# GoatWu/AdaLog

Measured on AMD Instinct MI355X. Metric: calib_images_per_sec, higher is better.
Workload: dtype bf16

## Files before the change

### adalog_amd/csrc/gemm_k_avw.inc

```
struct AvwCand { float s, inv, lo, hi; };
__device__ __forceinline__ uint4 avw_gen8(const v4u& xa, const v4u& xb, const AvwCand& c) {
#pragma clang fp contract(off)
    const float x[8] = {__uint_as_float(xa.x), __uint_as_float(xa.y), __uint_as_float(xa.z), __uint_as_float(xa.w),
                        __uint_as_float(xb.x), __uint_as_float(xb.y), __uint_as_float(xb.z), __uint_as_float(xb.w)};
    float k[8], dm = 0.0f;
#pragma unroll
    for (int e = 0; e < 8; ++e) {
        const float t = x[e] * c.inv;
        k[e] = rintf(t);
        dm = fmaxf(dm, fabsf(t - k[e]));
    }
    if (__builtin_expect(dm > 0.4999f, 0)) {
#pragma unroll
        for (int e = 0; e < 8; ++e) k[e] = rintf(x[e] / c.s);
    }
    uint32_t w[4];
#pragma unroll
    for (int e = 0; e < 4; ++e) {
        const uint32_t v0 = __float_as_uint(__builtin_amdgcn_fmed3f(k[2 * e], c.lo, c.hi));
        const uint32_t v1 = __float_as_uint(__builtin_amdgcn_fmed3f(k[2 * e + 1], c.lo, c.hi));
        w[e] = __builtin_amdgcn_perm(v1, v0, 0x07060302u);
    }
    return make_uint4(w[0], w[1], w[2], w[3]);
}

template <int NJ, bool R7>
__global__ __launch_bounds__(NJ * 64, 2) void k_gemm_avw_gen(GemmArgs p) {
#if defined(__HIP_DEVICE_COMPILE__)
    constexpr int NKS = 13, ASL = 25, ARB = ASL * 16, NT = NJ * 64, LA = 2;
    extern __shared__ __attribute__((aligned(16))) uint8_t lds[];
    const int tid = threadIdx.x, lane = tid & 63;
    const int w = __builtin_amdgcn_readfirstlane(tid >> 6);
    const int frow = lane & 31, fkg = lane >> 5;
    const int M = p.M, KbA = (int)p.KbA;
    const int nrb = R7 ? 7 : (M + 31) >> 5;
    const int NB = p.N >> 5;
    const int CB = p.slab_R, NCH = p.slab_U;
    const int items = p.G * NCH;
    const int ci = w * 32 + frow;
    double* wacc = p.wg_acc + (int64_t)blockIdx.x * p.gmod * 256;
    for (int i = tid; i < p.gmod * 256; i += NT) wacc[i] = 0.0;

    const int base0 = frow * ARB + fkg * 32, base6 = min(192 + frow, M) * ARB + fkg * 32;
    auto aoff = [&](int rb) { return R7 ? (rb < 6 ? base0 + rb * 32 * ARB : base6) : min(rb * 32 + frow, M) * ARB + fkg * 32; };
    const int xvoff = fkg * 64;

    for (int item = blockIdx.x; item < items; item += gridDim.x) {
        const int g = item / NCH, c = item - g * NCH, gh = g % p.gmod;
        const int blk0 = c * CB, nblk = min(CB, NB - blk0);
        const int d0 = blk0 / NJ, nd = nblk / NJ;
        __syncthreads();
        {
            const uint8_t* ag = p.A + (int64_t)g * p.sAg;
            const int nsl = min(ASL, KbA >> 4);
            for (int idx = tid; idx < (M + 1) * ASL + 4; idx += NT) {
                const int r = idx / ASL, s = idx - r * ASL;
                uint4 v = make_uint4(0, 0, 0, 0);
                if (r < M && s < nsl) v = *reinterpret_cast<const uint4*>(ag + (int64_t)r * KbA + s * 16);
                *reinterpret_cast<uint4*>(lds + r * ARB + s * 16) = v;
            }
        }
        __syncthreads();

        AvwCand cand;
        {
            const int64_t pi = ci * p.sb_c + gh * p.sb_g;
            const float z = rintf(p.gen_zp[pi]);
            cand.s = p.sb[pi]; cand.inv = __builtin_amdgcn_rcpf(cand.s); cand.lo = -z; cand.hi = p.gen_qmax - z;
        }
        const float nal = -(p.sa[ci * p.sa_c + gh * p.sa_g] * p.sa_mul * p.sb[ci * p.sb_c + gh * p.sb_g]);
        const int64_t xbytes = ((int64_t)(p.N / (NJ * 32)) * p.gen_ldx) * 4;
        const __amdgpu_buffer_rsrc_t rx = __builtin_amdgcn_make_buffer_rsrc((void*)(p.gen_x + (int64_t)g * p.gen_sg), 0,
                                                                            (int)min(xbytes, (int64_t)0x7ffffffe), 0x00020000);
        const float* refg = p.ref + (int64_t)g * p.sRg;
        auto load_x = [&](int d, int i, v4u& xa, v4u& xb) {
            const int so = d * (int)p.gen_ldx * 4;
            xa = __builtin_amdgcn_raw_buffer_load_b128(rx, xvoff + (32 * (i >> 1) + 8 * (i & 1)) * 4, so, 0);
            xb = __builtin_amdgcn_raw_buffer_load_b128(rx, xvoff + (32 * (i >> 1) + 8 * (i & 1)) * 4 + 16, so, 0);
        };
        auto load_a = [&](int i, uint4 (&af)[7]) {
#pragma unroll
            for (int rb = 0; rb < 7; ++rb)
                if (R7 || rb < nrb) af[rb] = *reinterpret_cast<const uint4*>(lds + aoff(rb) + (i >> 1) * 64 + (i & 1) * 16);
        };
        auto load_ref = [&](int d, int rb, float (&r)[16]) {
            const float* rp = refg + (int64_t)d * p.ref_cs;
#pragma unroll
            for (int q = 0; q < 4; ++q) {
                const int rr = rb * 32 + 8 * q + 4 * fkg;
                if (rr + 4 <= M) {
#pragma unroll
                    for (int e = 0; e < 4; ++e) r[4 * q + e] = rp[rr + e];
                } else {
#pragma unroll
                    for (int e = 0; e < 4; ++e) r[4 * q + e] = rr + e < M ? rp[rr + e] : 0.0f;
                }
            }
        };

        v2f csr[7];
#pragma unroll
        for (int rb = 0; rb < 7; ++rb) csr[rb] = (v2f){0.0f, 0.0f};

        v4u xq[NKS + LA][2];
#pragma unroll
        for (int i = 0; i < LA; ++i) load_x(d0, i, xq[i][0], xq[i][1]);
        for (int dd = 0; dd < nd; ++dd) {
            const int d = d0 + dd, dn = d0 + min(dd + 1, nd - 1);
            v16f acc[7];
#pragma unroll
            for (int rb = 0; rb < 7; ++rb)
#pragma unroll
                for (int e = 0; e < 16; ++e) acc[rb][e] = 0.0f;
            uint4 bq = avw_gen8(xq[0][0], xq[0][1], cand);
#pragma unroll
            for (int i = 0; i < NKS; ++i) {
                uint4 af[7];
                load_a(i, af);
                if (i + LA < NKS) load_x(d, i + LA, xq[i + LA][0], xq[i + LA][1]);
                else load_x(dn, i + LA - NKS, xq[i + LA][0], xq[i + LA][1]);
                uint4 bn = bq;
                if (i + 1 < NKS) bn = avw_gen8(xq[i + 1][0], xq[i + 1][1], cand);
                if (i + 1 == 12 && fkg) bn = make_uint4(0, 0, 0, 0);
#pragma unroll
                for (int rb = 0; rb < 7; ++rb)
                    if (R7 || rb < nrb) mma<1>(af[rb], bq, acc[rb]);
                bq = bn;
                __builtin_amdgcn_sched_barrier(0);
            }
#pragma unroll
            for (int i = 0; i < LA; ++i) { xq[i][0] = xq[NKS + i][0]; xq[i][1] = xq[NKS + i][1]; }
            float rc[16], rn[16];
            load_ref(d, 0, rc);
#pragma unroll
            for (int rb = 0; rb < 7; ++rb) {
                if (R7 || rb < nrb) {
                    if (rb + 1 < 7 && (R7 || rb + 1 < nrb)) load_ref(d, rb + 1, rn);
#pragma unroll
                    for (int q = 0; q < 4; ++q) {
                        const float e0 = __builtin_fmaf(acc[rb][q * 4 + 0], nal, rc[q * 4 + 0]);
                        const float e1 = __builtin_fmaf(acc[rb][q * 4 + 1], nal, rc[q * 4 + 1]);
                        const float e2 = __builtin_fmaf(acc[rb][q * 4 + 2], nal, rc[q * 4 + 2]);
                        const float e3 = __builtin_fmaf(acc[rb][q * 4 + 3], nal, rc[q * 4 + 3]);
                        csr[rb].x = __builtin_fmaf(e0, e0, csr[rb].x); csr[rb].y = __builtin_fmaf(e1, e1, csr[rb].y);
                        csr[rb].x = __builtin_fmaf(e2, e2, csr[rb].x); csr[rb].y = __builtin_fmaf(e3, e3, csr[rb].y);
                    }
#pragma unroll
                    for (int e = 0; e < 16; ++e) rc[e] = rn[e];
                }
            }
        }
        double v = 0.0;
#pragma unroll
        for (int rb = 0; rb < 7; ++rb) {
            if (R7 || rb < nrb) {
                float cs = csr[rb].x + csr[rb].y;
                cs += __shfl_xor(cs, 32);
                v += (double)cs;
            }
        }
        if (fkg == 0) wacc[gh * 256 + ci] += v;
    }
#endif
}
```

### adalog_amd/csrc/gemm_score.hip

```cpp
#include "common.h"
#include "fpcs_tail.h"
#include <stdlib.h>

#pragma clang fp contract(fast)

namespace {

#include "gemm_types.inc"
#include "gemm_k_basic.inc"
#include "gemm_k_stream.inc"
#include "gemm_k_slab.inc"
#include "gemm_k_grp.inc"
#include "gemm_k_avw.inc"
#include "gemm_finish.inc"

}

static int device_cus() {
    static int n_cu = 0;
    if (!n_cu) {
        int dev = 0; hipDeviceProp_t prop;
        if (hipGetDevice(&dev) == hipSuccess && hipGetDeviceProperties(&prop, dev) == hipSuccess) n_cu = prop.multiProcessorCount;
        if (n_cu <= 0) n_cu = 256;
    }
// ... 390 lines not shown
        p.slab_U = L.slab_U; p.slab_R = L.slab_R;
        const size_t shm = slab_lds(p.Kvb, L.slab_nb);
        if (!L.acc) {
            const hipError_t me = hipMemsetAsync(c.partial, 0, (size_t)L.elems * sizeof(float), st);
            if (me != hipSuccess) { adalog_set_error("adalog_gemm_score (clear partials)", me); return (int)me; }
        }
        e = with_slab(dtype, L.slab_nb, ref_div, [&](auto nr, auto dt, auto nb) {
            constexpr int NREF = decltype(nr)::value, DT = decltype(dt)::value, NB = decltype(nb)::value;
            return adalog_dispatch<true, false>(c.row_scale != nullptr, [&](auto rows) {
                return adalog_launch<k_gemm_slab<NREF, decltype(rows)::value, DT, NB>>(slab_label(0, DT, NB), 160 * 1024, wgs, 512, shm, st, p);
            });
        });
    } break;
    case R_WIN: {
        const size_t ref_lds = (size_t)4 * n_eff * 64 * 4, shm = ref_lds > acc_lds ? ref_lds : acc_lds;
        e = with_nj(ref_div, [&](auto nj) {
            constexpr int NJ = decltype(nj)::value;
            if (dtype == 3)
                return gen ? adalog_launch<k_gemm_win<NJ, 3, true>>("k_gemm_win_gen<fp8>", 80 * 1024, wgs, 256, shm, st, p)
                           : adalog_launch<k_gemm_win<NJ, 3>>("k_gemm_win<fp8>", 80 * 1024, wgs, 256, shm, st, p);
            return gen ? adalog_launch<k_gemm_win<NJ, 0, true>>("k_gemm_win_gen<i8>", 80 * 1024, wgs, 256, shm, st, p)
                       : adalog_launch<k_gemm_win<NJ, 0>>("k_gemm_win<i8>", 80 * 1024, wgs, 256, shm, st, p);
        });
    } break;
    case R_GRPW: {
        wave_chunks(p, n_eff, L.wgs, G);
        const size_t ref_lds = (size_t)4 * 2 * 224 * 4, shm = ref_lds > acc_lds ? ref_lds : acc_lds;
        e = with_nj(ref_div, [&](auto nj) {
            constexpr int NJ = decltype(nj)::value;
            if (dtype == 3)
                return gen ? adalog_launch<k_gemm_grpw<NJ, 3, true>>("k_gemm_grpw_gen<fp8>", 0, wgs, 256, shm, st, p)
                           : adalog_launch<k_gemm_grpw<NJ, 3>>("k_gemm_grpw<fp8>", 0, wgs, 256, shm, st, p);
            return gen ? adalog_launch<k_gemm_grpw<NJ, 0, true>>("k_gemm_grpw_gen<i8>", 0, wgs, 256, shm, st, p)
                       : adalog_launch<k_gemm_grpw<NJ, 0>>("k_gemm_grpw<i8>", 0, wgs, 256, shm, st, p);
        });
    } break;
    case R_GRP: {
        grp_chunks(p, N, L.wgs, G);
        const size_t shm = (size_t)3 * 8 * 32 * BK3 + 7 * 256 * 4 + acc_lds;
        e = with_nj(ref_div, [&](auto nj) {
            constexpr int NJ = decltype(nj)::value;
            return dtype == 3 ? adalog_launch<k_gemm_grp<NJ, 3>>("k_gemm_grp<fp8>", 96 * 1024, wgs, 512, shm, st, p)
                              : adalog_launch<k_gemm_grp<NJ, 0>>("k_gemm_grp<i8>", 96 * 1024, wgs, 512, shm, st, p);
        });
    } break;
    case R_GRPK: {
        grp_chunks(p, N, L.wgs, G);
        const size_t shm = (size_t)3 * 7 * 2 * 32 * BK3 + (size_t)7 * ref_div * 4 + acc_lds;
        e = with_nj(ref_div, [&](auto nj) {
            return adalog_launch<k_gemm_grpk<decltype(nj)::value, 7>>("k_gemm_grpk<bf16>", 160 * 1024, wgs, 512, shm, st, p);
        });
    } break;
    case R_STREAM: {
        p.gm = stream_gm(L, p.Kb);
        const size_t shm = (size_t)(L.wide ? 4 : 3) * (64 * L.tm + BN2) * BK3;
        e = adalog_dispatch<0, 1, 2, 3>(dtype, [&](auto dt) {
            return adalog_dispatch<4, 3, 2, 1>(L.wide ? L.wide : L.tm, [&](auto ri) {
                constexpr int DT = decltype(dt)::value, RI = decltype(ri)::value, NW = RI >= 3 ? 8 : 4, NS = RI >= 3 ? 4 : 3;
                return adalog_launch<k_gemm_stream<DT, RI, NW, NS>>(
                    DT == 0 ? "k_gemm_stream<i8>" : DT == 1 ? "k_gemm_stream<bf16>" : DT == 2 ? "k_gemm_stream<f32>" : "k_gemm_stream<fp8>",
                    (NS == 4 ? 128 : 80) * 1024, wgs, 64 * NW, shm, st, p);
            });
        });
    } break;
    case R_GLDS: {
        const size_t shm = (size_t)3 * (64 * L.tm + BN2) * BK2 + (512 + 256) * sizeof(float);
        e = adalog_dispatch<0, 1, 2>(dtype, [&](auto dt) {
            return adalog_dispatch<2, 1>(L.tm, [&](auto tm) {
                return adalog_launch<k_gemm_cand_glds<decltype(dt)::value, decltype(tm)::value>>("k_gemm_cand_glds", 160 * 1024, grid, 512, shm, st, p);
            });
        });
    } break;
    case R_CAND: {
        const size_t shm = (size_t)(64 * L.tm + BN2) * BK2 + (512 + 256) * sizeof(float);
        if (c.out && c.ox) ADALOG_ARG_CHECK(dtype == 0 || dtype == 1, "gemm_out_ex: int8 or bf16 operands");
        e = adalog_dispatch<4, 2, 1>(L.tm, [&](auto tm) {
            constexpr int TM = decltype(tm)::value;
            if (c.out && c.ox)
                return adalog_dispatch<0, 1>(dtype, [&](auto dt) {
                    return adalog_launch<k_gemm_cand<decltype(dt)::value, TM, true, false, true>>("k_gemm_cand_ex", 72 * 1024, grid, 512, shm, st, p);
                });
            return adalog_dispatch<0, 1, 2>(dtype, [&](auto dt) {
                return adalog_dispatch<true, false>(c.out != nullptr, [&](auto store) {
                    return adalog_launch<k_gemm_cand<decltype(dt)::value, TM, decltype(store)::value>>("k_gemm_cand", 72 * 1024, grid, 512, shm, st, p);
                });
            });
        });
    } break;
    default: {
        ADALOG_ARG_CHECK(!c.row_scale, "gemm_score: per-row scale is only available with C == 1");
        e = adalog_dispatch<0, 1, 2>(dtype, [&](auto dt) {
            return adalog_dispatch<true, false>(c.out != nullptr, [&](auto store) {
                return adalog_launch<k_gemm_score<decltype(dt)::value, decltype(store)::value>>("k_gemm_score", 0, grid, 256, 0, st, p);
            });
        });
    } break;
    }
    if (e) return e;
    ADALOG_LAUNCH_CHECK("adalog_gemm_score");
    return 0;
}

extern "C" int adalog_gemm_score(int dtype, const void* A, const void* B, int64_t sAc, int64_t sAg, int64_t sBc,
                                 int64_t sBg, int M, int N, int64_t Kp, int64_t k_valid, int C, int G, int gmod, const float* ref,
                                 int64_t ldr, int64_t sRg, int64_t ref_cs, int ref_div, const float* sa, int64_t sa_c,
                                 int64_t sa_g, float sa_mul, const float* sb, int64_t sb_c, int64_t sb_g, int64_t sb_n,
                                 const float* bias, int64_t bi_c, int64_t bi_g, int64_t bi_n, const float* row_scale,
                                 const float* row_bias, float* partial, int64_t partial_elems, float* out, int64_t ldo,
                                 int64_t sOc, int64_t sOg, int order, int reduce_cols, void* stream) {
    MmCall c{};
    c.dtype = dtype; c.A = A; c.B = B; c.sAc = sAc; c.sAg = sAg; c.sBc = sBc; c.sBg = sBg;
    c.M = M; c.N = N; c.Kp = Kp; c.k_valid = k_valid; c.C = C; c.G = G; c.gmod = gmod;
    c.ref = ref; c.ldr = ldr; c.sRg = sRg; c.ref_cs = ref_cs; c.ref_div = ref_div;
    c.sa = sa; c.sa_c = sa_c; c.sa_g = sa_g; c.sa_mul = sa_mul;
    c.sb = sb; c.sb_c = sb_c; c.sb_g = sb_g; c.sb_n = sb_n;
    c.bias = bias; c.bi_c = bi_c; c.bi_g = bi_g; c.bi_n = bi_n;
    c.row_scale = row_scale; c.row_bias = row_bias;
    c.partial = partial; c.partial_elems = partial_elems;
    c.out = out; c.ldo = ldo; c.sOc = sOc; c.sOg = sOg;
    c.order = order; c.reduce_cols = reduce_cols; c.stream = stream;
    return gemm_score_impl(c);
}

extern "C" int adalog_gemm_out_ex(int dtype, const void* A, const void* B, int64_t sAg, int64_t sBg, int M, int N, int64_t Kp, int G,
                                  int gmod, const float* sa, int64_t sa_g, float sa_mul, const float* sb, int64_t sb_g, int64_t sb_n,
                                  const float* bias, int64_t bi_g, int64_t bi_n, const float* addend, float* out, int64_t ldo,
                                  int64_t sOg, int out_gi, int64_t sOo, void* stream) {
    ADALOG_ARG_CHECK(out && (dtype == 0 || dtype == 1), "gemm_out_ex: int8 or bf16 operands, out required");
    const MmOutEx ox{addend, out_gi, sOo};
    MmCall c{};
    c.dtype = dtype; c.A = A; c.B = B; c.sAg = sAg; c.sBg = sBg;
    c.M = M; c.N = N; c.Kp = Kp; c.C = 1; c.G = G; c.gmod = gmod; c.ref_cs = 1; c.ref_div = 1;
    c.sa = sa; c.sa_g = sa_g; c.sa_mul = sa_mul;
    c.sb = sb; c.sb_g = sb_g; c.sb_n = sb_n;
    c.bias = bias; c.bi_g = bi_g; c.bi_n = bi_n;
    c.out = out; c.ldo = ldo; c.sOg = sOg; c.stream = stream; c.ox = &ox;
    return gemm_score_impl(c);
}


struct MmGenA { const float* x; int64_t ldx, sxg; int K; const float *a_scale, *a_zp; int64_t a_pg; int n_bits; const int *a_rows, *o_rows; int64_t period; };

static int gemm_out_gen_impl(const MmCall& c, const MmGenA& g) {
    const float *x = g.x, *a_scale = g.a_scale, *a_zp = g.a_zp, *addend = c.ox->addend;
    const int64_t ldx = g.ldx, Kp = c.Kp;
    const int K = g.K, n_bits = g.n_bits, M = c.M, N = c.N, G = c.G, gmod = c.gmod;
    const void* B = c.B;
    ADALOG_ARG_CHECK(x && a_scale && a_zp && B && c.sa && c.sb && c.out, "gemm_out_gen: null pointer");
    ADALOG_ARG_CHECK(M >= 1 && N >= 1 && G >= 1 && gmod >= 1 && G % gmod == 0 && K >= 16 && K % 16 == 0 && Kp >= K && Kp % BK2 == 0,
                     "gemm_out_gen: K must be a multiple of 16, Kp a multiple of 128 covering it");
    ADALOG_ARG_CHECK(n_bits >= 2 && n_bits <= 7 && ldx >= K && ldx % 4 == 0 && g.sxg % 4 == 0 && (((uintptr_t)x) & 15) == 0 &&
                     (((uintptr_t)B) & 15) == 0, "gemm_out_gen: <= 7-bit quantiser, 16-byte aligned fp32 rows");
    ADALOG_ARG_CHECK((int64_t)M * ldx < ((int64_t)1 << 31) && (int64_t)N * Kp < ((int64_t)1 << 31), "gemm_out_gen: operand exceeds 32-bit addressing");
    int tmv = pick_tm_out(M, (int64_t)cdiv(N, BN2) * G);
    if (tmv > 2) tmv = 2;
    Layout L{};
    L.MT = cdiv(M, 64 * tmv); L.NT = cdiv(N, BN2); L.Npad = L.NT * BN2;
    GemmArgs p = gemm_args(c, L);
    p.KbA = Kp; p.timeline = nullptr;
    p.gen_x = x; p.gen_ldx = ldx; p.gen_sg = g.sxg; p.gen_K = K; p.gen_scale = a_scale; p.gen_zp = a_zp; p.gen_sn = g.a_pg;
    p.gen_qmax = (float)((1 << n_bits) - 1);
    const bool rowmap = g.a_rows || g.o_rows;
    p.a_rows = g.a_rows; p.o_rows = g.o_rows; p.row_period = (int)(rowmap ? g.period : 1);
    const int64_t tiles = (int64_t)p.MT * p.NT * G;
    ADALOG_ARG_CHECK(tiles < ((int64_t)1 << 31), "gemm_out_gen: grid too large");
    const size_t shm = (size_t)(64 * tmv + BN2) * BK2 + (512 + 256) * sizeof(float);
    const char* label = rowmap ? "k_gemm_cand_gen_rows" : addend ? "k_gemm_cand_gen_ex" : "k_gemm_cand_gen";
    if (const int e = adalog_dispatch<true, false>(rowmap, [&](auto map) {
            return adalog_dispatch<true, false>(addend != nullptr, [&](auto add) {
                return adalog_dispatch<2, 1>(tmv, [&](auto tm) {
                    return adalog_launch<k_gemm_cand<0, decltype(tm)::value, true, true, decltype(add)::value, decltype(map)::value>>(
                        label, 72 * 1024, (unsigned)tiles, 512, shm, (hipStream_t)c.stream, p);
                });
            });
        })) return e;
    ADALOG_LAUNCH_CHECK("adalog_gemm_out_gen");
    return 0;
}

extern "C" int adalog_gemm_out_gen(const float* x, int64_t ldx, int64_t sxg, int K, const float* a_scale, const float* a_zp, int64_t a_pg,
                                   int n_bits, const void* B, int64_t sBg, int M, int N, int64_t Kp, int G, int gmod, const float* sa,
                                   int64_t sa_g, float sa_mul, const float* sb, int64_t sb_g, int64_t sb_n, const float* bias,
                                   int64_t bi_g, int64_t bi_n, const float* addend, float* out, int64_t ldo, int64_t sOg, void* stream) {
    const MmOutEx ox{addend, 0, 0};
    const MmGenA g{x, ldx, sxg, K, a_scale, a_zp, a_pg, n_bits, nullptr, nullptr, 1};
    MmCall c{};
    c.B = B; c.sBg = sBg; c.M = M; c.N = N; c.Kp = Kp; c.k_valid = K; c.C = 1; c.G = G; c.gmod = gmod; c.ref_cs = 1; c.ref_div = 1;
    c.sa = sa; c.sa_g = sa_g; c.sa_mul = sa_mul; c.sb = sb; c.sb_g = sb_g; c.sb_n = sb_n; c.bias = bias; c.bi_g = bi_g; c.bi_n = bi_n;
    c.out = out; c.ldo = ldo; c.sOg = sOg; c.stream = stream; c.ox = &ox;
    return gemm_out_gen_impl(c, g);
}

extern "C" int adalog_gemm_out_gen_rows(const float* x, int64_t ldx, int K, const float* a_scale, const float* a_zp, int n_bits,
                                        const void* B, int M, int N, int64_t Kp, const float* sa, float sa_mul, const float* sb,
                                        int64_t sb_n, const float* bias, int64_t bi_n, const float* addend, float* out, int64_t ldo,
                                        const int* a_rows, const int* o_rows, int64_t period, void* stream) {
    ADALOG_ARG_CHECK(period >= 1 && M % period == 0, "gemm_out_gen_rows: M must be a multiple of the period");
    ADALOG_ARG_CHECK(ldo >= N && (int64_t)M * ldo < ((int64_t)1 << 31), "gemm_out_gen_rows: output exceeds 32-bit addressing");
    const MmOutEx ox{addend, 0, 0};
    const MmGenA g{x, ldx, 0, K, a_scale, a_zp, 0, n_bits, a_rows, o_rows, period};
    MmCall c{};
    c.B = B; c.M = M; c.N = N; c.Kp = Kp; c.k_valid = K; c.C = 1; c.G = 1; c.gmod = 1; c.ref_cs = 1; c.ref_div = 1;
    c.sa = sa; c.sa_mul = sa_mul; c.sb = sb; c.sb_n = sb_n; c.bias = bias; c.bi_n = bi_n;
    c.out = out; c.ldo = ldo; c.stream = stream; c.ox = &ox;
    return gemm_out_gen_impl(c, g);
}

extern "C" int adalog_gemm_score_gen(int dtype, const void* A, int64_t sAg, int M, int N, int64_t Kp, int64_t k_valid, int G, int gmod,
                                     const float* x, int64_t ldx, int64_t sg, const float* zp, int n_bits, const float* ref,
                                     int64_t sRg, int ref_div, const float* sa, int64_t sa_c, int64_t sa_g, float sa_mul,
                                     const float* sb, int64_t sb_c, int64_t sb_g, float* partial, int64_t partial_elems,
                                     void* stream) {
    ADALOG_ARG_CHECK(n_bits >= 1 && n_bits <= 8 && (dtype != 3 || n_bits <= 4), "gemm_score_gen: fp8 candidates hold <= 4-bit values");
    const MmGen gen{x, ldx, sg, zp, n_bits};
    MmCall c{};
    c.dtype = dtype; c.A = A; c.sAg = sAg; c.M = M; c.N = N; c.Kp = Kp; c.k_valid = k_valid; c.C = 1; c.G = G; c.gmod = gmod;
    c.ref = ref; c.ldr = 1; c.sRg = sRg; c.ref_cs = M; c.ref_div = ref_div;
    c.sa = sa; c.sa_c = sa_c; c.sa_g = sa_g; c.sa_mul = sa_mul; c.sb = sb; c.sb_c = sb_c; c.sb_g = sb_g;
    c.partial = partial; c.partial_elems = partial_elems; c.order = 2; c.reduce_cols = 1; c.stream = stream; c.gen = &gen;
    return gemm_score_impl(c);
}

static Layout av_layout(int M, int N, int G, int gmod, int P, int64_t k_valid, int64_t Kp) {
    return layout_of(M, N * P, 1, G, gmod, P, 1, true, k_valid * 2, Kp * 2, true, 1);
}
static GemmArgs av_gen_args(const void* A, int64_t sAg, int M, int N, int64_t k_valid, int G, int gmod, const float* x, int64_t ldx,
                            int64_t sg, const float* ref, int64_t sRg, int P, const float* sa, int64_t sa_c, int64_t sa_g, float sa_mul,
                            const float* sb, int64_t sb_c, int64_t sb_g, float* partial) {
    GemmArgs p{};
    p.A = (const uint8_t*)A; p.sAg = sAg * 2; p.M = M; p.N = N * P; p.C = 1; p.G = G; p.gmod = gmod;
    p.ref = ref; p.ldr = 1; p.sRg = sRg; p.ref_cs = M; p.ref_div = P;
    p.sa = sa; p.sa_c = sa_c; p.sa_g = sa_g; p.sa_mul = sa_mul; p.sb = sb; p.sb_c = sb_c; p.sb_g = sb_g;
    p.wg_acc = (double*)partial; p.partial = partial; p.gen_x = x; p.gen_ldx = ldx; p.gen_sg = sg; p.gen_K = (int)k_valid;
    return p;
}

static bool avq_ok(int M, int N, int G, int gmod, int P, int64_t k_valid, int64_t Kp, int n_bits, Layout* L = nullptr) {
    static const int use_avq = getenv("ADALOG_GEMM_AVQ") ? atoi(getenv("ADALOG_GEMM_AVQ")) : 1;
    if (!use_avq || P != 128 || M < 1 || M > 64 || N < 1 || k_valid < 1 || k_valid > 208 || n_bits < 1 || n_bits > 6 || gmod < 1 || gmod > 16 ||
        G % gmod || G < 8)
        return false;
    const int nks = k_valid <= 64 ? 4 : 13;
    if (Kp < nks * 16 || (Kp * 2) % 16) return false;
    const Layout l = av_layout(M, N, G, gmod, P, k_valid, Kp);
    if (L) *L = l;
    return l.stream && l.acc && !l.slab && l.wgs * 4 >= gmod;
}
extern "C" int adalog_gemm_score_avq_ok(int M, int N, int G, int gmod, int P, int64_t k_valid, int64_t Kp, int n_bits) {
    return avq_ok(M, N, G, gmod, P, k_valid, Kp, n_bits) ? 1 : 0;
}
extern "C" int adalog_gemm_score_avq(const void* A, int64_t sAg, int M, int N, int64_t Kp, int64_t k_valid, int G, int gmod,
                                     const float* x, int64_t ldx, int64_t sg, const float* q, const uint32_t* lut, int n_bits,
                                     const float* ref, int64_t sRg, int P, const float* sa, int64_t sa_c, int64_t sa_g, float sa_mul,
                                     const float* sb, int64_t sb_c, int64_t sb_g, float* partial, int64_t partial_elems,
                                     void* stream) {
    ADALOG_ARG_CHECK(A && x && q && lut && ref && sa && sb && partial, "gemm_score_avq: null pointer");
    Layout L{};
    ADALOG_ARG_CHECK(avq_ok(M, N, G, gmod, P, k_valid, Kp, n_bits, &L), "gemm_score_avq: shape not taken (adalog_gemm_score_avq_ok)");
    ADALOG_ARG_CHECK((((uintptr_t)A) & 15) == 0 && (((uintptr_t)partial) & 7) == 0, "gemm_score_avq: operand / accumulator alignment");
    ADALOG_ARG_CHECK(partial_elems >= L.elems, "gemm_score_avq: partial buffer too small");
    GemmArgs p = av_gen_args(A, sAg, M, N, k_valid, G, gmod, x, ldx, sg, ref, sRg, P, sa, sa_c, sa_g, sa_mul, sb, sb_c, sb_g, partial);
    p.Kb = Kp * 2; p.Kvb = k_valid * 2; p.gen_q = q; p.gen_lut = lut; p.gen_nb = 1 << n_bits;
    wave_chunks(p, N, L.wgs, G, cdiv(N, AVQ_ROWS));
    const int nks = k_valid <= 64 ? 4 : 13;
    const size_t lut_b = (((size_t)(p.gen_nb + 1) * P + 3) & ~(size_t)3) * 4;
    const size_t rows_b = (size_t)4 * ((size_t)AVQ_ROWS * (nks * 16 + 64) + 4 * 64 * 2) * 4;
    const size_t acc_b = (size_t)gmod * 256 * 8;
    const size_t shm = lut_b + rows_b > acc_b ? lut_b + rows_b : acc_b;
    hipStream_t st = (hipStream_t)stream;
    const unsigned wgs = (unsigned)L.wgs;
    const int e = nks == 13 ? (M > 32 ? adalog_launch<k_gemm_avq<4, 13, 2>>("k_gemm_avq<13,bf16>", 80 * 1024, wgs, 256, shm, st, p)
                                      : adalog_launch<k_gemm_avq<4, 13, 1>>("k_gemm_avq<13,bf16>", 80 * 1024, wgs, 256, shm, st, p))
                            : (M > 32 ? adalog_launch<k_gemm_avq<4, 4, 2>>("k_gemm_avq<4,bf16>", 80 * 1024, wgs, 256, shm, st, p)
                                      : adalog_launch<k_gemm_avq<4, 4, 1>>("k_gemm_avq<4,bf16>", 80 * 1024, wgs, 256, shm, st, p));
    if (e) return e;
    ADALOG_LAUNCH_CHECK("adalog_gemm_score_avq");
    return 0;
}

static int avw_wgs(int M, int N, int G, int gmod, int P, int64_t k_valid, int64_t Kp, int n_bits) {
    if (!(P == 64 || P == 128 || P == 256) || M < 1 || M > 224 || N < 32 || N % 32 || k_valid < 1 || k_valid > 200 || Kp < k_valid || Kp % 8 ||
        n_bits < 1 || n_bits > 4 || gmod < 1 || G < 1 || G % gmod || (int64_t)N * P >= ((int64_t)1 << 30))
        return 0;
    const Layout L = av_layout(M, N, G, gmod, P, k_valid, Kp);
    return (L.stream && L.acc && !L.slab && L.wgs >= 1) ? L.wgs : 0;
}
extern "C" int adalog_gemm_score_avw_ok(int M, int N, int G, int gmod, int P, int64_t k_valid, int64_t Kp, int n_bits) {
    return avw_wgs(M, N, G, gmod, P, k_valid, Kp, n_bits);
}
extern "C" int adalog_gemm_score_avw(const void* A, int64_t sAg, int M, int N, int64_t Kp, int64_t k_valid, int G, int gmod,
                                     const float* x, int64_t ldx, int64_t sg, const float* zp, int n_bits, const float* ref, int64_t sRg,
                                     int P, const float* sa, int64_t sa_c, int64_t sa_g, float sa_mul, const float* sb, int64_t sb_c,
                                     int64_t sb_g, float* partial, int64_t partial_elems, void* stream) {
    ADALOG_ARG_CHECK(A && x && zp && ref && sa && sb && partial, "gemm_score_avw: null pointer");
    const int wgs = avw_wgs(M, N, G, gmod, P, k_valid, Kp, n_bits);
    ADALOG_ARG_CHECK(wgs > 0, "gemm_score_avw: shape not taken (adalog_gemm_score_avw_ok)");
    ADALOG_ARG_CHECK((((uintptr_t)A) & 15) == 0 && (sAg * 2) % 16 == 0 && (((uintptr_t)partial) & 7) == 0 && (((uintptr_t)x) & 3) == 0,
                     "gemm_score_avw: operand / accumulator alignment");
    ADALOG_ARG_CHECK(ldx >= k_valid && (int64_t)N * ldx * 4 < ((int64_t)1 << 31), "gemm_score_avw: rows of x shorter than K, or a group of x beyond 32-bit addressing");
    ADALOG_ARG_CHECK(partial_elems >= (int64_t)2 * wgs * gmod * BN2, "gemm_score_avw: partial buffer too small");
    GemmArgs p = av_gen_args(A, sAg, M, N, k_valid, G, gmod, x, ldx, sg, ref, sRg, P, sa, sa_c, sa_g, sa_mul, sb, sb_c, sb_g, partial);
    p.Kb = Kp; p.KbA = Kp * 2; p.Kvb = k_valid; p.gen_zp = zp; p.gen_qmax = (float)((1 << n_bits) - 1);
    grp_chunks(p, N * P, wgs, G);
    const size_t shm = (size_t)(M + 1) * 400 + 64;
    hipStream_t st = (hipStream_t)stream;
    if (const int e = with_nj(P, [&](auto nj) {
            constexpr int NJ = decltype(nj)::value;
            return M > 192 ? adalog_launch<k_gemm_avw_gen<NJ, true>>("k_gemm_avw_gen<13,bf16>", 160 * 1024, (unsigned)wgs, NJ * 64, shm, st, p)
                           : adalog_launch<k_gemm_avw_gen<NJ, false>>("k_gemm_avw_gen<13,bf16>", 160 * 1024, (unsigned)wgs, NJ * 64, shm, st, p);
        })) return e;
    ADALOG_LAUNCH_CHECK("adalog_gemm_score_avw");
    return 0;
}

extern "C" int adalog_gemm_score_gen_ok(int dtype, int M, int N, int G, int gmod, int ref_div, int64_t k_valid, int64_t Kp) {
    if (!(dtype == 0 || dtype == 3) || k_valid < 16 || k_valid > 64 || k_valid % 16 || ref_div < 1 || N % ref_div != 0 || G % gmod) return 0;
    const MmCall c = shape_call(dtype, M, N, G, gmod, ref_div, k_valid, Kp, 1);
    const Route r = route_of(c, call_layout(c, true));
    return (r == R_WIN || r == R_GRPW) ? 1 : 0;
}

static GemmArgs slab_gen_args(const Layout& L, const void* A, int rows, int64_t cols, int64_t Kp, const float* x, int64_t ldx, int K,
                              const float* scale, const float* zp, int P, int n_bits, const float* ref, float* partial) {
    GemmArgs p{};
    p.A = (const uint8_t*)A; p.M = rows; p.N = (int)(cols * P); p.Kb = Kp; p.Kvb = K; p.C = 1; p.G = 1; p.gmod = 1;
    p.ref = ref; p.ldr = 1; p.ref_cs = rows; p.ref_div = P; p.sa_mul = 1.0f; p.sb = scale;
    p.MT = L.MT; p.NT = L.NT; p.Npad = L.Npad; p.order = 2; p.reduce_cols = 0; p.timeline = g_timeline;
    p.partial = partial; p.slab_U = L.slab_U; p.slab_R = L.slab_R;
    p.gen_x = x; p.gen_ldx = ldx; p.gen_K = K; p.gen_scale = scale; p.gen_zp = zp; p.gen_qmax = (float)((1 << n_bits) - 1);
    const float zone = 6e-7f * (float)(1 << n_bits);
    p.gen_tie = 0.5f - (zone > 1e-5f ? zone : 1e-5f);
    return p;
}
template <bool SCORE_ACT>
static int slab_gen_launch(int form, int dtype, const Layout& L, int P, hipStream_t st, const GemmArgs& p) {
    const size_t shm = slab_lds(p.Kvb, L.slab_nb);
    return with_slab(dtype, L.slab_nb, P, [&](auto nr, auto dt, auto nb) {
        constexpr int NREF = decltype(nr)::value, DT = decltype(dt)::value, NB = decltype(nb)::value;
        return adalog_launch<k_gemm_slab<NREF, SCORE_ACT, DT, NB, true>>(slab_label(form, DT, NB), 160 * 1024, (unsigned)L.wgs, 512, shm, st, p);
    });
}

static Layout gen_layout(int dtype, int M, int64_t T, int K, int64_t Kp, int P) {
    Layout L{};
    if (!(dtype == 0 || dtype == 3) || !(P == 64 || P == 128 || P == 256) || T < 1 || T * P >= ((int64_t)1 << 31) || K < 16 || K % 16 != 0 ||
        Kp < K) return L;
    return layout_of(M, (int)(T * P), 1, 1, 1, P, 1, true, (int64_t)K, Kp, true, dtype, true);
}

extern "C" int adalog_score_act_gen_ok(int dtype, int M, int64_t T, int K, int64_t Kp, int P) {
    static const int use_gen = getenv("ADALOG_SLAB_GEN") ? atoi(getenv("ADALOG_SLAB_GEN")) : 1;
    if (!use_gen || Kp % BK3 != 0) return 0;
    const Layout L = gen_layout(dtype, M, T, K, Kp, P);
    return (L.slab && L.acc) ? 1 : 0;
}

extern "C" int adalog_score_act_gen_wgs(int dtype, int M, int64_t T, int K, int64_t Kp, int P) {
    const Layout L = gen_layout(dtype, M, T, K, Kp, P);
    return (L.slab && L.acc) ? L.wgs : -1;
}

extern "C" int64_t adalog_score_act_gen_workspace_bytes(int dtype, int M, int64_t T, int K, int64_t Kp, int P) {
    const Layout L = gen_layout(dtype, M, T, K, Kp, P);
    if (!(L.slab && L.acc)) return -1;
    return L.elems * (int64_t)sizeof(float) + ((int64_t)M * 4 + 15) / 16 * 16;
}

extern "C" int adalog_score_act_gen(int dtype, const void* Wp, int M, int64_t Kp, const float* x, int64_t T, int K, int64_t ldx,
                                    const float* scale, const float* zp, int P, int n_bits, const float* ref,
                                    const float* row_scale, const float* row_bias, double norm, void* workspace,
                                    int64_t workspace_bytes, float* scores, void* stream) {
    ADALOG_ARG_CHECK(Wp && x && scale && zp && ref && row_scale && workspace, "score_act_gen: null pointer");
    ADALOG_ARG_CHECK(n_bits >= 2 && n_bits <= 7 && (dtype != 3 || n_bits <= 4), "score_act_gen: bad bit width for the operand type");
    ADALOG_ARG_CHECK(ldx >= K && (ldx % 4 == 0) && ((uintptr_t)x & 15) == 0, "score_act_gen: activation rows must be 16-byte aligned");
    const Layout L = gen_layout(dtype, M, T, K, Kp, P);
    ADALOG_ARG_CHECK(L.slab && L.acc && Kp % BK3 == 0, "score_act_gen: shape not taken by the slab kernel (adalog_score_act_gen_ok)");
    ADALOG_ARG_CHECK(workspace_bytes >= adalog_score_act_gen_workspace_bytes(dtype, M, T, K, Kp, P) && ((uintptr_t)workspace & 15) == 0,
                     "score_act_gen: workspace too small or misaligned");
    hipStream_t st = (hipStream_t)stream;
    float* partial = (float*)workspace;
    float* zero_bias = (float*)((uint8_t*)workspace + L.elems * sizeof(float));
    if (!row_bias) {
        const hipError_t me = hipMemsetAsync(zero_bias, 0, (size_t)M * 4, st);
        if (me != hipSuccess) { adalog_set_error("adalog_score_act_gen (zero bias)", me); return (int)me; }
        row_bias = zero_bias;
    }
    GemmArgs p = slab_gen_args(L, Wp, M, T, Kp, x, ldx, K, scale, zp, P, n_bits, ref, partial);
    ADALOG_ARG_CHECK((int64_t)(T - 1) * M + M < ((int64_t)1 << 31), "score_act_gen: reference exceeds 32-bit addressing");
    p.sa = scale; p.sb_c = 1; p.row_scale = row_scale; p.row_bias = row_bias; p.wg_acc = (double*)partial; p.gen_sc = 1;
    if (const int e = slab_gen_launch<true>(1, dtype, L, P, st, p)) return e;
    ADALOG_LAUNCH_CHECK("adalog_score_act_gen");
    if (!scores) return 0;
    return adalog_finish_scores(partial, scores, L.wgs, BN2, BN2, P, 1, 1, 0, 0, 2, norm, nullptr, 0, stream);
}

static Layout wgen_layout(int dtype, int T, int O, int K, int64_t Kp, int P) {
    Layout L{};
    if (!(dtype == 0 || dtype == 3) || !(P == 64 || P == 128 || P == 256) || O < 1 || (int64_t)O * P >= ((int64_t)1 << 31) || K < 16 || K % 16 != 0 ||
        Kp < K) return L;
    return layout_of(T, O * P, 1, 1, 1, P, 0, true, (int64_t)K, Kp, true, dtype, false);
}

extern "C" int adalog_score_w_gen_ok(int dtype, int T, int O, int K, int64_t Kp, int P) {
    static const int use_gen = getenv("ADALOG_SLAB_WGEN") ? atoi(getenv("ADALOG_SLAB_WGEN")) : 1;
    if (!use_gen || Kp % BK3 != 0) return 0;
    const Layout L = wgen_layout(dtype, T, O, K, Kp, P);
    return (L.slab && !L.acc) ? 1 : 0;
}

extern "C" int adalog_score_w_gen(int dtype, const void* Xp, int T, int64_t Kp, const float* W, int O, int K, int64_t ldw,
                                  const float* scale, const float* zp, int P, int n_bits, const float* ref, const float* sa,
                                  const float* bias, float* partial, int64_t partial_elems, void* stream) {
    ADALOG_ARG_CHECK(Xp && W && scale && zp && ref && sa && partial, "score_w_gen: null pointer");
    ADALOG_ARG_CHECK(n_bits >= 2 && n_bits <= 7 && (dtype != 3 || n_bits <= 4), "score_w_gen: bad bit width for the operand type");
    ADALOG_ARG_CHECK(ldw >= K && (ldw % 4 == 0) && ((uintptr_t)W & 15) == 0, "score_w_gen: weight rows must be 16-byte aligned");
    const Layout L = wgen_layout(dtype, T, O, K, Kp, P);
    ADALOG_ARG_CHECK(L.slab && !L.acc && Kp % BK3 == 0, "score_w_gen: shape not taken by the slab kernel (adalog_score_w_gen_ok)");
    ADALOG_ARG_CHECK(partial_elems >= L.elems, "score_w_gen: partial buffer too small");
    hipStream_t st = (hipStream_t)stream;
    GemmArgs p = slab_gen_args(L, Xp, T, O, Kp, W, ldw, K, scale, zp, P, n_bits, ref, partial);
    ADALOG_ARG_CHECK((int64_t)(O - 1) * T + T < ((int64_t)1 << 31), "score_w_gen: reference exceeds 32-bit addressing");
    p.sa = sa; p.sb_c = O; p.sb_n = 1; p.bias = bias; p.bi_n = 1; p.gen_sc = O; p.gen_sn = 1; p.gen_sa = sa;
    {
        const hipError_t me = hipMemsetAsync(partial, 0, (size_t)L.elems * sizeof(float), st);
        if (me != hipSuccess) { adalog_set_error("adalog_score_w_gen (clear partials)", me); return (int)me; }
    }
    if (const int e = slab_gen_launch<false>(2, dtype, L, P, st, p)) return e;
    ADALOG_LAUNCH_CHECK("adalog_score_w_gen");
    return 0;
}

extern "C" int64_t adalog_finish_workspace_bytes(int MT, int N, int C, int G, int keep_n, int cand_inner) {
    if (cand_inner != 1 || keep_n || !(C == 64 || C == 128 || C == 256)) return 0;
    return (int64_t)G * MT * cdiv(N, FSEG) * C * (int64_t)sizeof(double);
}

extern "C" int adalog_finish_scores(const float* partial, float* scores, int MT, int N, int Npad, int C, int G, int gmod,
                                    int keep_h, int keep_n, int cand_inner, double norm, void* workspace,
                                    int64_t workspace_bytes, void* stream) {
    ADALOG_ARG_CHECK(partial && scores && MT >= 1 && N >= 1 && Npad >= N && C >= 1 && G >= 1 && gmod >= 1 && G % gmod == 0,
                     "finish_scores: bad arguments");
    FinishArgs p{};
    p.partial = partial; p.scores = scores; p.C = C; p.G = G; p.gmod = gmod; p.MT = MT; p.N = N; p.Npad = Npad;
    p.keep_h = keep_h; p.keep_n = keep_n; p.norm = norm; p.cin = cand_inner ? C : 0;
    if (cand_inner == 2) {
        ADALOG_ARG_CHECK(!keep_n && (C == 64 || C == 128 || C == 256) && Npad == 256, "finish_scores: bad accumulator layout");
        const int64_t nout2 = (int64_t)C * (keep_h ? gmod : 1);
        hipLaunchKernelGGL(k_finish_wgacc, dim3((unsigned)nout2), dim3(256), 0, (hipStream_t)stream, p,
                           (const double*)partial, MT);
        ADALOG_LAUNCH_CHECK("adalog_finish_scores");
        return 0;
    }
    const int64_t nout = (int64_t)C * (keep_h ? gmod : 1) * (keep_n ? N : 1);
    const int64_t per_out = (int64_t)(G / gmod) * (keep_h ? 1 : gmod) * MT * (keep_n ? 1 : N);
    const int64_t need = adalog_finish_workspace_bytes(MT, N, C, G, keep_n, cand_inner);
    if (need > 0 && workspace && workspace_bytes >= need && per_out >= 1024) {
        const int nseg = cdiv(N, FSEG);
        hipLaunchKernelGGL(k_finish_rows, dim3((unsigned)nseg, (unsigned)(G * MT)), dim3(256), 0, (hipStream_t)stream, p,
                           (double*)workspace, nseg);
        hipLaunchKernelGGL(k_finish_stage2, dim3((unsigned)((nout + 3) / 4)), dim3(256), 0, (hipStream_t)stream, p,
                           (const double*)workspace, nseg);
    } else if (p.cin > 0 && per_out <= 512 && nout >= 4096)
        hipLaunchKernelGGL(k_finish_tpo, dim3((unsigned)((nout + 255) / 256)), dim3(256), 0, (hipStream_t)stream, p);
    else if (per_out >= 2048)
        hipLaunchKernelGGL(k_finish<false>, dim3((unsigned)nout), dim3(256), 0, (hipStream_t)stream, p);
    else
        hipLaunchKernelGGL(k_finish<true>, dim3((unsigned)((nout + 3) / 4)), dim3(256), 0, (hipStream_t)stream, p);
    ADALOG_LAUNCH_CHECK("adalog_finish_scores");
    return 0;
}

extern "C" int adalog_finish_topk_next_tail(const float* partial, float* scores, int MT, int N, int Npad, int C, int G, int gmod,
                                            int keep_h, int keep_n, int cand_inner, double norm, void* workspace, int64_t workspace_bytes,
                                            const adalog_fpcs_tail* tail, void* stream) {
    ADALOG_ARG_CHECK(partial && scores && tail && MT >= 1 && N >= 1 && Npad >= N && C >= 1 && C <= 256 && G >= 1 &&
                     gmod >= 1 && G % gmod == 0, "finish_topk_next: bad arguments");
    const char* why = fpcs::tail_problem(tail, C);
    ADALOG_ARG_CHECK(why == nullptr, why);
    static const int use_fused = getenv("ADALOG_FINISH_TOPK") ? atoi(getenv("ADALOG_FINISH_TOPK")) : 1;
    const int nh = keep_h ? gmod : 1, nn = keep_n ? N : 1, cols = nh * nn;
    FinishArgs p{};
    p.partial = partial; p.scores = scores; p.C = C; p.G = G; p.gmod = gmod; p.MT = MT; p.N = N; p.Npad = Npad;
    p.keep_h = keep_h; p.keep_n = keep_n; p.norm = norm; p.cin = cand_inner ? C : 0;
    const TopkArgs t = *tail;
    hipStream_t st = (hipStream_t)stream;
    const bool c_ok = (C == 64 || C == 128 || C == 256);
    if (use_fused && cand_inner == 2 && !keep_n && c_ok && Npad == 256 && nh <= 64) {
        unsigned int* ticket = adalog_ticket_slots_on(nh, stream);
        if (ticket) {
            hipLaunchKernelGGL(k_finish_wgacc_topk, dim3((unsigned)(C * nh)), dim3(256), 0, st, p, (const double*)partial, MT, t, ticket);
            ADALOG_LAUNCH_CHECK("adalog_finish_topk_next");
            return 0;
        }
    }
    const int64_t nout = (int64_t)C * cols;
    const int64_t per_out = (int64_t)(G / gmod) * (keep_h ? 1 : gmod) * MT * (keep_n ? 1 : N);
    if (use_fused && cand_inner == 1 && c_ok && per_out <= 512 && nout >= 4096) {
        const int gpb = 256 / C;
        hipLaunchKernelGGL(k_finish_tpo_topk, dim3((unsigned)((cols + gpb - 1) / gpb)), dim3(256), 0, st, p, t);
        ADALOG_LAUNCH_CHECK("adalog_finish_topk_next");
        return 0;
    }
    const int rc = adalog_finish_scores(partial, scores, MT, N, Npad, C, G, gmod, keep_h, keep_n, cand_inner, norm, workspace,
                                        workspace_bytes, stream);
    if (rc) return rc;
    return adalog_topk_next_tail(scores, C, cols, tail, nullptr, stream);
}

extern "C" int adalog_finish_topk_next(const float* partial, float* scores, int MT, int N, int Npad, int C, int G, int gmod,
                                       int keep_h, int keep_n, int cand_inner, double norm, void* workspace, int64_t workspace_bytes,
                                       int k, const float* scale, const float* zp, const float* third, int new_cnt,
                                       const float* lin, float* delta, int has_clamp, float clamp_min, float* out_scale,
                                       float* out_zp, float* out_third, void* stream) {
    const adalog_fpcs_tail t{k, new_cnt, has_clamp, clamp_min, scale, zp, third, lin, delta, delta, out_scale, out_zp, out_third};
    return adalog_finish_topk_next_tail(partial, scores, MT, N, Npad, C, G, gmod, keep_h, keep_n, cand_inner, norm, workspace,
                                        workspace_bytes, &t, stream);
}
```

Before: 38.15.

## Stage reference rows in LDS with double buffering and batch the A-tile load

Reference values are now fetched cooperatively (coalesced per thread) into LDS, double-buffered across output columns when LDS capacity allows, and read back as float4 from LDS in the epilogue instead of as scattered per-lane global loads. The A-tile staging loop is unrolled to issue ten independent global loads before the LDS stores, and the image is padded to a multiple of 32 rows so the row clamp in aoff can be dropped. In exchange it adds __syncthreads per column and more LDS use, which may reduce occupancy.

```diff
diff --git a/adalog_amd/csrc/gemm_k_avw.inc b/adalog_amd/csrc/gemm_k_avw.inc
--- a/adalog_amd/csrc/gemm_k_avw.inc
+++ b/adalog_amd/csrc/gemm_k_avw.inc
@@ -1,3 +1,8 @@
+constexpr int AVW_REF_BYTES = 224 * 4;
+__host__ __device__ constexpr int avw_img_rows(int M) { return M > 192 ? M : (M + 31) & ~31; }
+__host__ __device__ constexpr int avw_img_bytes(int M) { return (avw_img_rows(M) + 1) * 400 + 64; }
+__host__ __device__ constexpr bool avw_ref_two(int M) { return 2 * (avw_img_bytes(M) + 2 * AVW_REF_BYTES) <= 160 * 1024; }
+__host__ __device__ constexpr int avw_lds_bytes(int M) { return avw_img_bytes(M) + (avw_ref_two(M) ? 2 : 1) * AVW_REF_BYTES; }
 struct AvwCand { float s, inv, lo, hi; };
 __device__ __forceinline__ uint4 avw_gen8(const v4u& xa, const v4u& xb, const AvwCand& c) {
 #pragma clang fp contract(off)
@@ -28,6 +33,8 @@
 __global__ __launch_bounds__(NJ * 64, 2) void k_gemm_avw_gen(GemmArgs p) {
 #if defined(__HIP_DEVICE_COMPILE__)
     constexpr int NKS = 13, ASL = 25, ARB = ASL * 16, NT = NJ * 64, LA = 2;
+    constexpr int IU = 10;
+    constexpr int RPT = (224 + NT - 1) / NT;
     extern __shared__ __attribute__((aligned(16))) uint8_t lds[];
     const int tid = threadIdx.x, lane = tid & 63;
     const int w = __builtin_amdgcn_readfirstlane(tid >> 6);
@@ -42,23 +49,55 @@
     for (int i = tid; i < p.gmod * 256; i += NT) wacc[i] = 0.0;
 
     const int base0 = frow * ARB + fkg * 32, base6 = min(192 + frow, M) * ARB + fkg * 32;
-    auto aoff = [&](int rb) { return R7 ? (rb < 6 ? base0 + rb * 32 * ARB : base6) : min(rb * 32 + frow, M) * ARB + fkg * 32; };
+    auto aoff = [&](int rb) { return rb < 6 ? base0 + rb * 32 * ARB : base6; };
     const int xvoff = fkg * 64;
+    const int ir0 = tid / ASL, is0 = tid - ir0 * ASL;
+    const int islots = (avw_img_rows(M) + 1) * ASL + 4;
+    const int nsl = min(ASL, KbA >> 4);
+    const int refo = avw_img_bytes(M) + fkg * 16;
+    const bool two = avw_ref_two(M);
 
     for (int item = blockIdx.x; item < items; item += gridDim.x) {
         const int g = item / NCH, c = item - g * NCH, gh = g % p.gmod;
         const int blk0 = c * CB, nblk = min(CB, NB - blk0);
         const int d0 = blk0 / NJ, nd = nblk / NJ;
+        const float* refg = p.ref + (int64_t)g * p.sRg;
+        auto ref_fetch = [&](int d, float (&r)[RPT]) {
+            const float* rp = refg + (int64_t)d * p.ref_cs;
+#pragma unroll
+            for (int u = 0; u < RPT; ++u) {
+                const int t = tid + u * NT;
+                r[u] = t < M ? rp[t] : 0.0f;
+            }
+        };
+        auto ref_put = [&](int b, const float (&r)[RPT]) {
+#pragma unroll
+            for (int u = 0; u < RPT; ++u) {
+                const int t = tid + u * NT;
+                if (t < 224) *reinterpret_cast<float*>(lds + avw_img_bytes(M) + b * AVW_REF_BYTES + t * 4) = r[u];
+            }
+        };
         __syncthreads();
         {
             const uint8_t* ag = p.A + (int64_t)g * p.sAg;
-            const int nsl = min(ASL, KbA >> 4);
-            for (int idx = tid; idx < (M + 1) * ASL + 4; idx += NT) {
-                const int r = idx / ASL, s = idx - r * ASL;
-                uint4 v = make_uint4(0, 0, 0, 0);
-                if (r < M && s < nsl) v = *reinterpret_cast<const uint4*>(ag + (int64_t)r * KbA + s * 16);
-                *reinterpret_cast<uint4*>(lds + r * ARB + s * 16) = v;
-            }
+            float r0[RPT];
+            ref_fetch(d0, r0);
+            int r = ir0, s = is0;
+            for (int idx = tid; idx < islots; idx += IU * NT) {
+                uint4 v[IU];
+#pragma unroll
+                for (int u = 0; u < IU; ++u) {
+                    const bool in = r < M && s < nsl;
+                    v[u] = *reinterpret_cast<const uint4*>(ag + (in ? r * KbA + s * 16 : 0));
+                    if (!in) v[u] = make_uint4(0, 0, 0, 0);
+                    r += NT / ASL; s += NT % ASL;
+                    if (s >= ASL) { s -= ASL; ++r; }
+                }
+#pragma unroll
+                for (int u = 0; u < IU; ++u)
+                    if (idx + u * NT < islots) *reinterpret_cast<uint4*>(lds + (idx + u * NT) * 16) = v[u];
+            }
+            ref_put(0, r0);
         }
         __syncthreads();
 
@@ -72,7 +111,6 @@
         const int64_t xbytes = ((int64_t)(p.N / (NJ * 32)) * p.gen_ldx) * 4;
         const __amdgpu_buffer_rsrc_t rx = __builtin_amdgcn_make_buffer_rsrc((void*)(p.gen_x + (int64_t)g * p.gen_sg), 0,
                                                                             (int)min(xbytes, (int64_t)0x7ffffffe), 0x00020000);
-        const float* refg = p.ref + (int64_t)g * p.sRg;
         auto load_x = [&](int d, int i, v4u& xa, v4u& xb) {
             const int so = d * (int)p.gen_ldx * 4;
             xa = __builtin_amdgcn_raw_buffer_load_b128(rx, xvoff + (32 * (i >> 1) + 8 * (i & 1)) * 4, so, 0);
@@ -83,18 +121,11 @@
             for (int rb = 0; rb < 7; ++rb)
                 if (R7 || rb < nrb) af[rb] = *reinterpret_cast<const uint4*>(lds + aoff(rb) + (i >> 1) * 64 + (i & 1) * 16);
         };
-        auto load_ref = [&](int d, int rb, float (&r)[16]) {
-            const float* rp = refg + (int64_t)d * p.ref_cs;
+        auto load_ref = [&](int b, int rb, float (&r)[16]) {
 #pragma unroll
             for (int q = 0; q < 4; ++q) {
-                const int rr = rb * 32 + 8 * q + 4 * fkg;
-                if (rr + 4 <= M) {
-#pragma unroll
-                    for (int e = 0; e < 4; ++e) r[4 * q + e] = rp[rr + e];
-                } else {
-#pragma unroll
-                    for (int e = 0; e < 4; ++e) r[4 * q + e] = rr + e < M ? rp[rr + e] : 0.0f;
-                }
+                const float4 t = *reinterpret_cast<const float4*>(lds + refo + b * AVW_REF_BYTES + (rb * 32 + 8 * q) * 4);
+                r[4 * q + 0] = t.x; r[4 * q + 1] = t.y; r[4 * q + 2] = t.z; r[4 * q + 3] = t.w;
             }
         };
 
@@ -107,6 +138,8 @@
         for (int i = 0; i < LA; ++i) load_x(d0, i, xq[i][0], xq[i][1]);
         for (int dd = 0; dd < nd; ++dd) {
             const int d = d0 + dd, dn = d0 + min(dd + 1, nd - 1);
+            float rnx[RPT];
+            if (two && dd + 1 < nd) ref_fetch(d + 1, rnx);
             v16f acc[7];
 #pragma unroll
             for (int rb = 0; rb < 7; ++rb)
@@ -130,12 +163,22 @@
             }
 #pragma unroll
             for (int i = 0; i < LA; ++i) { xq[i][0] = xq[NKS + i][0]; xq[i][1] = xq[NKS + i][1]; }
-            float rc[16], rn[16];
-            load_ref(d, 0, rc);
+            int rbuf = 0;
+            if (two) {
+                __syncthreads();
+                if (dd + 1 < nd) ref_put((dd + 1) & 1, rnx);
+                rbuf = dd & 1;
+            } else if (dd > 0) {
+                __syncthreads();
+                ref_fetch(d, rnx);
+                ref_put(0, rnx);
+                __syncthreads();
+            }
 #pragma unroll
             for (int rb = 0; rb < 7; ++rb) {
                 if (R7 || rb < nrb) {
-                    if (rb + 1 < 7 && (R7 || rb + 1 < nrb)) load_ref(d, rb + 1, rn);
+                    float rc[16];
+                    load_ref(rbuf, rb, rc);
 #pragma unroll
                     for (int q = 0; q < 4; ++q) {
                         const float e0 = __builtin_fmaf(acc[rb][q * 4 + 0], nal, rc[q * 4 + 0]);
@@ -145,8 +188,6 @@
                         csr[rb].x = __builtin_fmaf(e0, e0, csr[rb].x); csr[rb].y = __builtin_fmaf(e1, e1, csr[rb].y);
                         csr[rb].x = __builtin_fmaf(e2, e2, csr[rb].x); csr[rb].y = __builtin_fmaf(e3, e3, csr[rb].y);
                     }
-#pragma unroll
-                    for (int e = 0; e < 16; ++e) rc[e] = rn[e];
                 }
             }
         }
diff --git a/adalog_amd/csrc/gemm_score.hip b/adalog_amd/csrc/gemm_score.hip
--- a/adalog_amd/csrc/gemm_score.hip
+++ b/adalog_amd/csrc/gemm_score.hip
@@ -716,7 +716,7 @@
     GemmArgs p = av_gen_args(A, sAg, M, N, k_valid, G, gmod, x, ldx, sg, ref, sRg, P, sa, sa_c, sa_g, sa_mul, sb, sb_c, sb_g, partial);
     p.Kb = Kp; p.KbA = Kp * 2; p.Kvb = k_valid; p.gen_zp = zp; p.gen_qmax = (float)((1 << n_bits) - 1);
     grp_chunks(p, N * P, wgs, G);
-    const size_t shm = (size_t)(M + 1) * 400 + 64;
+    const size_t shm = (size_t)avw_lds_bytes(M);
     hipStream_t st = (hipStream_t)stream;
     if (const int e = with_nj(P, [&](auto nj) {
             constexpr int NJ = decltype(nj)::value;
```

Result: faster. 39.69, median of 6 (+4.0%).
